# Byshx/Poccala

Hardware: AMD Instinct MI355X
Metric: frames/sec GMM-score+fwd-bwd, 39-d MFCC, 2048-mix (higher is better)
Workload: dtype f32-class (f16x2 split operands, f32 accumulate; f64 dynamic programming)

## Files before the change

### poccala_amd/csrc/batch_plan.h

```cpp
#pragma once
#include <math.h>
#include <stdint.h>

#include <algorithm>
#include <vector>

#include "pcl_own.h"

struct ScoreSeg {
    long long frame0;
    long long out0;
    int len;
    int out_stride;
    int vstart;
    int pad;
};
struct DupRow {
    long long src, dst;
    int T, N;
};
struct ScoreTile {
    int state;
    int seg_lo, seg_hi;
    int vstart;
// ... 119 lines not shown

template <typename Rows>
static int plan_sparse_trans(pcl_ctx *ctx, const char *who, std::vector<UttDesc> &utt, Rows rows, SparseTrans *out) {
    SparseTrans s;
    size_t np = 0;
    for (const UttDesc &d : utt) np += (size_t)d.N + 1;
    s.row_ptr.resize(np);
    s.col_ptr.resize(np);
    std::vector<int> nnz_off(utt.size()), fill;
    for (size_t u = 0; u < utt.size(); ++u) {
        const UttDesc &d = utt[u];
        const int N = d.N;
        const size_t base = s.col_idx.size();
        nnz_off[u] = (int)base;
        int *rp = s.row_ptr.data() + d.ptr_off, *cp = s.col_ptr.data() + d.ptr_off;
        for (int i = 0; i < N; ++i) {
            rp[i] = (int)(s.col_idx.size() - base);
            rows((int)u, i, [&](int j, double v) {
                s.col_idx.push_back(j);
                s.csr_val.push_back(v);
                if (j != i && j != i + 1) s.shape.left_right = false;
            });
            s.shape.max_outdeg = std::max(s.shape.max_outdeg, (int)(s.col_idx.size() - base) - rp[i]);
        }
        if (s.col_idx.size() > 0x7fffffffULL) PCL_FAIL(ctx, PCL_ERR_INVALID, "%s: too many transitions", who);
        const int cnt = rp[N] = (int)(s.col_idx.size() - base);
        std::fill(cp, cp + N + 1, 0);
        for (int k = 0; k < cnt; ++k) ++cp[s.col_idx[base + k] + 1];
        for (int j = 0; j < N; ++j) {
            s.shape.max_indeg = std::max(s.shape.max_indeg, cp[j + 1]);
            cp[j + 1] += cp[j];
        }
        fill.assign(cp, cp + N);
        s.row_idx.resize(base + cnt);
        s.csc_val.resize(base + cnt);
        for (int i = 0; i < N; ++i)
            for (int k = rp[i]; k < rp[i + 1]; ++k) {
                const int q = fill[s.col_idx[base + k]]++;
                s.row_idx[base + q] = i;
                s.csc_val[base + q] = s.csr_val[base + k];
            }
    }
    s.shape.nnz = (long long)s.col_idx.size();
    for (size_t u = 0; u < utt.size(); ++u) utt[u].nnz_off = nnz_off[u];
    *out = std::move(s);
    return PCL_OK;
}

static auto dense_trans_rows(const std::vector<UttDesc> &utt, const double *logA) {
    return [&utt, logA](int u, int i, auto emit) {
        const int N = utt[u].N;
        const double *row = logA + utt[u].mat_off + (size_t)i * N;
        for (int j = 0; j < N; ++j)
            if (!(row[j] == -INFINITY)) emit(j, row[j]);
    };
}
static auto label_trans_rows(const std::vector<UttDesc> &utt, const LabelPlan &lab, const double *unit_logtrans, int S) {
    return [&utt, &lab, unit_logtrans, S](int u, int i, auto emit) {
        if (i == utt[u].N - 1) return;
        const int e = S - 2, p = (i == 0) ? 0 : (i - 1) / e, r = (i == 0) ? 0 : 1 + (i - 1) % e;
        const double *row = unit_logtrans + ((size_t)lab.labels[lab.label_off[u] + p] * S + r) * S;
        for (int c = 0; c < S; ++c)
            if (!(row[c] == -INFINITY)) emit(p * e + c, row[c]);
    };
}

struct ScorePlan {
    std::vector<int32_t> row_state;
    std::vector<ScoreSeg> segs;
    std::vector<DupRow> dups;
    std::vector<int> seg_of_row;
    std::vector<int> work_states;
    std::vector<int> state_seg_lo, state_seg_hi;
    std::vector<int> state_seg_hip;
    int n_segs = 0;
    int max_state = -1;
    int max_N = 0;
};

static int plan_score(pcl_ctx *ctx, const std::vector<UttDesc> &utt, const int32_t *row_state, int J, ScorePlan *out) {
    const int U = (int)utt.size();
    ScorePlan p;
    std::vector<int> start((size_t)J + 1, 0);
    std::vector<long long> frames(J, 0);
    size_t sumN = 0;
    for (int u = 0; u < U; ++u) {
        const UttDesc &d = utt[u];
        for (int n = 0; n < d.N; ++n) {
            const int st = row_state[d.vec_off + n];
            if (st >= J || st < PCL_ROW_EXIT) PCL_FAIL(ctx, PCL_ERR_INVALID, "pcl_batch_set_states: utterance %d row %d has state %d outside [0,%d)", u, n, st, J);
            if (st < 0) continue;
            if (d.frame0 < 0) PCL_FAIL(ctx, PCL_ERR_STATE, "pcl_batch_set_states: batch was created without frame_begin");
            if ((frames[st] += d.T) > 0x7fffffffLL) PCL_FAIL(ctx, PCL_ERR_INVALID, "pcl_batch_set_states: state %d has too many frames", st);
            ++start[st + 1];
            p.max_state = std::max(p.max_state, st);
        }
        sumN += d.N;
        p.max_N = std::max(p.max_N, d.N);
    }
    for (int j = 0; j < J; ++j) start[j + 1] += start[j];
    p.n_segs = start[J];
    p.row_state.assign(row_state, row_state + sumN);
    std::vector<int> nprim(J, 0), first_row(J, -1), touched;
    std::vector<char> is_dup(sumN, 0);
    for (int u = 0; u < U; ++u) {
        const UttDesc &d = utt[u];
        touched.clear();
        for (int n = 0; n < d.N; ++n) {
            const int st = row_state[d.vec_off + n];
            if (st < 0) continue;
            if (first_row[st] < 0) {
                first_row[st] = n;
                touched.push_back(st);
                ++nprim[st];
            } else {
                is_dup[d.vec_off + n] = 1;
                p.dups.push_back(DupRow{d.b_off + first_row[st], d.b_off + n, d.T, d.N});
            }
        }
        for (int st : touched) first_row[st] = -1;
    }
    p.segs.assign(p.n_segs, ScoreSeg());
    p.seg_of_row.assign(sumN, -1);
    std::vector<int> fill(start.begin(), start.end() - 1);
    std::fill(frames.begin(), frames.end(), 0);
    for (int pass = 0; pass < 2; ++pass)
        for (int u = 0; u < U; ++u) {
            const UttDesc &d = utt[u];
            for (int n = 0; n < d.N; ++n) {
                const int st = row_state[d.vec_off + n];
                if (st < 0 || (int)is_dup[d.vec_off + n] != pass) continue;
                p.seg_of_row[d.vec_off + n] = fill[st];
                ScoreSeg &s = p.segs[fill[st]++];
                s.frame0 = d.frame0;
                s.out0 = d.b_off + n;
                s.len = d.T;
                s.out_stride = d.N;
                s.vstart = (int)frames[st];
                s.pad = st;
                frames[st] += d.T;
            }
        }
    for (int j = 0; j < J; ++j)
        if (start[j + 1] > start[j]) {
            p.work_states.push_back(j);
            p.state_seg_lo.push_back(start[j]);
            p.state_seg_hi.push_back(start[j + 1]);
            p.state_seg_hip.push_back(start[j] + nprim[j]);
        }
    *out = std::move(p);
    return PCL_OK;
}

static std::vector<ScoreTile> plan_tiles(const ScorePlan &p, const std::vector<size_t> &which, int tf) {
    constexpr int NXCD = 8;
    std::vector<ScoreTile> queue[NXCD];
    std::vector<long long> load(NXCD, 0);
    for (size_t k : which) {
        const int lo = p.state_seg_lo[k], hi = p.state_seg_hip[k];
        const long long tot = (long long)p.segs[hi - 1].vstart + p.segs[hi - 1].len;
        int g = 0;
        for (int x = 1; x < NXCD; ++x)
            if (load[x] < load[g]) g = x;
        int s0 = lo;
        for (long long v = 0; v < tot; v += tf) {
            while (s0 + 1 < hi && p.segs[s0 + 1].vstart <= v) ++s0;
            queue[g].push_back(ScoreTile{p.work_states[k], lo, hi, (int)v, s0});
        }
        load[g] += (tot + tf - 1) / tf;
    }
    size_t depth = 0;
    for (int x = 0; x < NXCD; ++x) depth = std::max(depth, queue[x].size());
    std::vector<ScoreTile> tiles;
    tiles.reserve(depth * NXCD);
    for (size_t q = 0; q < depth; ++q)
        for (int x = 0; x < NXCD; ++x) tiles.push_back(q < queue[x].size() ? queue[x][q] : ScoreTile{0, 0, 0, 0, 0});
    return tiles;
}
```

### poccala_amd/csrc/pcl_api.hip

```cpp
#include <math.h>
#include <stdio.h>
#include <stdlib.h>
#include <string.h>

#include <algorithm>

#include <map>
#include <memory>
#include <mutex>
#include <unordered_map>

#include "pcl_internal.h"

static std::string g_init_error;

void pcl_set_error(pcl_ctx *ctx, const char *msg) {
    if (ctx) ctx->err = msg;
    else g_init_error = msg;
}

void pcl_timer_begin(pcl_ctx *ctx, const char *which) {
    if (!ctx->timing) return;
    TimedEventPair p;
    if (p.make() != hipSuccess) return;
// ... 24 lines not shown
size_t pool_class(size_t n) {
    if (n <= 256) return 256;
    size_t p2 = 256;
    while (p2 < n) p2 <<= 1;
    if (p2 <= (1u << 20)) return p2;
    const size_t step = p2 >> 4;
    return (n + step - 1) / step * step;
}
size_t pool_limit() {
    static const size_t lim = (size_t)(getenv("PCL_POOL_MAX_MB") ? atol(getenv("PCL_POOL_MAX_MB")) : 65536) << 20;
    return lim;
}
void pool_release_locked(size_t keep) {
    while (g_pool_cached > keep && !g_pool_free.empty()) {
        auto best = g_pool_free.begin();
        for (auto it = g_pool_free.begin(); it != g_pool_free.end(); ++it)
            if (it->first.second > best->first.second) best = it;
        int cur = 0;
        (void)hipGetDevice(&cur);
        if (cur != best->first.first) (void)hipSetDevice(best->first.first);
        (void)hipFree(best->second);
        if (cur != best->first.first) (void)hipSetDevice(cur);
        g_pool_cached -= best->first.second;
        g_pool_live.erase(best->second);
        g_pool_free.erase(best);
    }
}
}

void *pcl_pool_alloc(int device, size_t bytes) {
    const size_t cls = pool_class(bytes);
    std::lock_guard<std::mutex> lock(g_pool_mu);
    auto it = g_pool_free.find(std::make_pair(device, cls));
    if (it != g_pool_free.end()) {
        void *p = it->second;
        g_pool_free.erase(it);
        g_pool_cached -= cls;
        return p;
    }
    void *p = nullptr;
    if (hipMalloc(&p, cls) != hipSuccess) {
        (void)hipGetLastError();
        pool_release_locked(0);
        if (hipMalloc(&p, cls) != hipSuccess) {
            (void)hipGetLastError();
            return nullptr;
        }
    }
    ++g_pool_device_allocs;
    g_pool_live[p] = PoolBlock{cls, device};
    return p;
}

void pcl_pool_free(void *p) {
    if (!p) return;
    const bool wait = pcl_tls_free_synced <= 0;
    if (wait) (void)hipDeviceSynchronize();
    std::lock_guard<std::mutex> lock(g_pool_mu);
    if (wait) ++g_pool_device_waits;
    auto it = g_pool_live.find(p);
    if (it == g_pool_live.end()) {
        (void)hipFree(p);
        return;
    }
    g_pool_free.emplace(std::make_pair(it->second.device, it->second.bytes), p);
    g_pool_cached += it->second.bytes;
    if (g_pool_cached > pool_limit()) pool_release_locked(pool_limit() / 2);
}

extern "C" int pcl_pool_stats(size_t *handed_out_blocks, size_t *handed_out_bytes, size_t *cached_bytes, uint64_t *device_allocs, uint64_t *device_waits) {
    std::lock_guard<std::mutex> lock(g_pool_mu);
    size_t live_bytes = 0;
    for (const auto &kv : g_pool_live) live_bytes += kv.second.bytes;
    if (handed_out_blocks) *handed_out_blocks = g_pool_live.size() - g_pool_free.size();
    if (handed_out_bytes) *handed_out_bytes = live_bytes - g_pool_cached;
    if (cached_bytes) *cached_bytes = g_pool_cached;
    if (device_allocs) *device_allocs = g_pool_device_allocs;
    if (device_waits) *device_waits = g_pool_device_waits;
    return PCL_OK;
}

namespace {
__global__ void desc_copy_kernel(DescCopyArgs a, const char *__restrict__ stage) {
    const int e = blockIdx.y;
    if (e >= a.n) return;
    const unsigned long long n = a.bytes[e];
    if (n == 0) return;
    const char *src = stage + a.off[e];
    char *dst = (char *)a.dst[e];
    const unsigned long long n16 = n / 16;
    for (unsigned long long i = blockIdx.x * (unsigned long long)blockDim.x + threadIdx.x; i < n16; i += (unsigned long long)gridDim.x * blockDim.x)
        ((uint4 *)dst)[i] = ((const uint4 *)src)[i];
    if (blockIdx.x == 0)
        for (unsigned long long i = n16 * 16 + threadIdx.x; i < n; i += blockDim.x) dst[i] = src[i];
}
}

hipError_t pcl_desc_launch(pcl_ctx *ctx, const DescCopyArgs &a, const char *pin) {
    void *dev_stage = nullptr;
    hipError_t e = hipHostGetDevicePointer(&dev_stage, const_cast<char *>(pin), 0);
    if (e != hipSuccess) return e;
    hipLaunchKernelGGL(desc_copy_kernel, dim3(32, a.n), dim3(256), 0, ctx->stream_desc, a, (const char *)dev_stage);
    e = hipGetLastError();
    return e != hipSuccess ? e : hipStreamSynchronize(ctx->stream_desc);
}

static int pcl_batch_reap(pcl_ctx *ctx, bool wait);

extern "C" {

static void free_model(pcl_ctx *ctx) {
    pcl_accumulate_release(ctx);
    pcl_coarse_release(ctx);
    ctx->nbad.clear();
    if (ctx->zero_pending && ctx->ev_zero) (void)hipEventSynchronize(ctx->ev_zero);
    ctx->zero_pending = false;
    static_cast<ModelDev &>(*ctx) = {};
    ctx->st_acc = ctx->st_alpha = ctx->st_mean = ctx->st_cov = nullptr;
    ctx->J = ctx->M = ctx->Mpad = 0;
}

static void release_frames32(pcl_ctx *ctx) {
    if (ctx->frames_front < 0) ctx->frames_up.release();
    ctx->frames32 = nullptr;
    ctx->frames_front = -1;
}

static int ctx_setup(pcl_ctx *ctx) {
    HIPCHK(nullptr, hipSetDevice(ctx->device));
    hipDeviceProp_t prop;
    if (hipGetDeviceProperties(&prop, ctx->device) == hipSuccess) ctx->cus = prop.multiProcessorCount;
    HIPCHK(nullptr, ctx->stream_main.make(StreamKind::Plain));
    ctx->stream = ctx->stream_main;
    HIPCHK(nullptr, ctx->stream_dp.make(StreamKind::HighPriority));
    HIPCHK(nullptr, ctx->stream_aux.make(StreamKind::Plain));
    HIPCHK(nullptr, ctx->stream_desc.make(StreamKind::NonBlocking));
    HIPCHK(nullptr, ctx->stream_d2h.make(StreamKind::NonBlocking));
    const char *var = getenv("PCL_SCORE_VARIANT");
    ctx->score_variant = var ? atoi(var) : 7;
    if (ctx->score_variant != 1 && ctx->score_variant != 3 && ctx->score_variant != 7)
        PCL_FAIL(nullptr, PCL_ERR_INVALID, "pcl_init: PCL_SCORE_VARIANT must be 1, 3 or 7");
    if (const char *cm = getenv("PCL_MFMA_COND_MAX")) ctx->cond_max = (float)atof(cm);
    if (const char *sm = getenv("PCL_SPLIT_MAX")) {
        ctx->split_frac = std::min(1.0f, std::max(0.0f, (float)atof(sm)));
        ctx->split_frac_set = true;
    }
    if (const char *ds = getenv("PCL_DP_STREAM")) ctx->dp_async = atoi(ds) != 0;
    if (const char *co = getenv("PCL_COARSE")) ctx->coarse_on = atoi(co) != 0;
    if (const char *cm2 = getenv("PCL_COMPACT_MAIN")) ctx->compact_main = atoi(cm2) != 0;
    if (const char *cs = getenv("PCL_COARSE_STATS")) ctx->coarse_stats = atoi(cs) != 0;
    if (const char *cp = getenv("PCL_COARSE_PASSES")) ctx->coarse_np = atoi(cp) == 3 ? 3 : 1;
    if (const char *cm_ = getenv("PCL_COARSE_SPLIT_MAX")) ctx->coarse_split_frac = std::min(1.0f, std::max(0.0f, (float)atof(cm_)));
    if (const char *tm = getenv("PCL_TIMERS")) ctx->timing = atoi(tm) != 0;
    return PCL_OK;
}

static void ctx_teardown(pcl_ctx *ctx) {
    pcl_comm_destroy(ctx);
    pcl_batch_reap(ctx, true);
    ctx->zero_pending = false;
    delete ctx;
}

int pcl_init(int device, pcl_ctx **out) {
    if (!out) PCL_FAIL(nullptr, PCL_ERR_INVALID, "pcl_init: out is NULL");
    *out = nullptr;
    setenv("GPU_MAX_HW_QUEUES", "8", 0);
    int n = 0;
    hipError_t e = hipGetDeviceCount(&n);
    if (e != hipSuccess || n == 0)
        PCL_FAIL(nullptr, PCL_ERR_HIP, "pcl_init: no HIP device (%s)", e == hipSuccess ? "count = 0" : hipGetErrorString(e));
    if (device < 0 || device >= n) PCL_FAIL(nullptr, PCL_ERR_INVALID, "pcl_init: device %d out of range [0,%d)", device, n);
    pcl_ctx *ctx = new pcl_ctx();
    ctx->device = device;
    const int rc = ctx_setup(ctx);
    if (rc != PCL_OK) {
        ctx_teardown(ctx);
        return rc;
    }
    *out = ctx;
    return PCL_OK;
}

int pcl_destroy(pcl_ctx *ctx) {
    if (!ctx) return PCL_OK;
    hipSetDevice(ctx->device);
    for (int round = 0; round < 2; ++round) {
        for (hipStream_t s : ctx->streams())
            if (s) hipStreamSynchronize(s);
    }
    ctx_teardown(ctx);
    return PCL_OK;
}

const char *pcl_last_error(pcl_ctx *ctx) { return ctx ? ctx->err.c_str() : g_init_error.c_str(); }

static int sync_main_and_dp(pcl_ctx *ctx) {
    HIPCHK(ctx, hipStreamSynchronize(ctx->stream));
    HIPCHK(ctx, hipStreamSynchronize(ctx->stream_dp));
    return PCL_OK;
}

int pcl_sync(pcl_ctx *ctx) {
    if (!ctx) return PCL_ERR_INVALID;
    TRY(sync_main_and_dp(ctx));
    HIPCHK(ctx, hipStreamSynchronize(ctx->stream_aux));
    if (ctx->stream_d2h) HIPCHK(ctx, hipStreamSynchronize(ctx->stream_d2h));
    pcl_batch_reap(ctx, false);
    return PCL_OK;
}

static int batch_join(pcl_batch *b) {
    if (b->dp_pending) {
        HIPCHK(b->ctx, hipStreamWaitEvent(b->ctx->stream, b->ev_dp, 0));
        b->dp_pending = false;
    }
    if (b->fetch_pending) {
        HIPCHK(b->ctx, hipStreamWaitEvent(b->ctx->stream, b->ev_fetch, 0));
        b->fetch_pending = false;
    }
    return PCL_OK;
}

int pcl_device_info(pcl_ctx *ctx, char *name, int cap, int *cus, size_t *hbm_bytes) {
    if (!ctx) return PCL_ERR_INVALID;
    hipDeviceProp_t prop;
    HIPCHK(ctx, hipGetDeviceProperties(&prop, ctx->device));
    if (name && cap > 0) snprintf(name, cap, "%s (%s)", prop.name, prop.gcnArchName);
    if (cus) *cus = prop.multiProcessorCount;
    if (hbm_bytes) *hbm_bytes = prop.totalGlobalMem;
    return PCL_OK;
}

int pcl_timing_enable(pcl_ctx *ctx, int on) {
    if (!ctx) return PCL_ERR_INVALID;
    TRY(sync_main_and_dp(ctx));
    if (!on) ctx->timers.clear();
    ctx->timing = on != 0;
    return PCL_OK;
}

int pcl_kernel_time(pcl_ctx *ctx, const char *which, float *total_ms, int *launches) {
    if (!ctx || !which) return PCL_ERR_INVALID;
    TRY(sync_main_and_dp(ctx));
    float tot = 0.f;
    int n = 0;
    auto it = ctx->timers.find(which);
    if (it != ctx->timers.end()) {
        for (auto &p : it->second.ev) {
            float ms = 0.f;
            if (hipEventElapsedTime(&ms, p.first, p.second) == hipSuccess) {
                tot += ms;
                ++n;
            }
        }
        it->second.ev.clear();
        tot += (float)it->second.host_ms;
        n += it->second.host_n;
        it->second.host_ms = 0.0;
        it->second.host_n = 0;
    }
    if (total_ms) *total_ms = tot;
    if (launches) *launches = n;
    return PCL_OK;
}

static int device_dim(int D) {
    const int pipe[] = {13, 26, 39, 47};
    for (int o : pipe)
        if (D <= o) return o;
    const int opts[] = {48, 64};
    for (int o : opts)
        if (D <= o) return o;
    return -1;
}

int pcl_device_dim(int D) { return device_dim(D); }

void pcl_frames_adopt(pcl_ctx *ctx, DevBuf<float> &&f32, DevBuf<double> &&f64, int64_t F, int D) {
    release_frames32(ctx);
    ctx->frames64.release();
    ctx->frames_up = std::move(f32);
    ctx->frames32 = ctx->frames_up;
    ctx->frames64 = std::move(f64);
    ctx->F = F;
    ctx->FD = device_dim(D);
    ctx->FDhost = D;
    if (ctx->fmllr_Gk && D != ctx->Dhost) pcl_fmllr_release(ctx);
    if (ctx->mllt_F && D != ctx->Dhost) pcl_mllt_release(ctx);
}

int pcl_model_alloc(pcl_ctx *ctx, int J, int M, int D, int flags, const char *who) {
    if (J <= 0 || M <= 0 || D <= 0) PCL_FAIL(ctx, PCL_ERR_INVALID, "%s: bad shape J=%d M=%d D=%d", who, J, M, D);
    const int Dd = device_dim(D);
    if (Dd < 0) PCL_FAIL(ctx, PCL_ERR_INVALID, "%s: feature dimension %d > 64 is not supported", who, D);
    HIPCHK(ctx, hipSetDevice(ctx->device));
    free_model(ctx);
    const int Mpad = (M + 3) / 4 * 4;
    const int row = (2 * Dd + 1 + 3) / 4 * 4;
    const int Mp32 = (M + 31) / 32 * 32, KS4 = (Dd + 1 + 3) / 4;
    const size_t nm = (size_t)J * Mpad * Dd, nw = (size_t)J * Mpad;
    const size_t npm = (size_t)J * (Mp32 / 32) * KS4 * 64 * 4;
    TRY(ctx->mean64.alloc(ctx, nm));
    TRY(ctx->var64.alloc(ctx, nm));
    TRY(ctx->w64.alloc(ctx, nw));
    TRY(ctx->pm32.alloc(ctx, npm));
// ... 228 lines not shown
    else ctx->graves.push_back(b);
    return PCL_OK;
}

int pcl_batch_upload_sparse(pcl_batch *b, const SparseTrans &t, const double *logpi) {
    pcl_ctx *ctx = b->ctx;
    b->trans = t.shape;
    b->row_ptr.release(); b->col_idx.release(); b->csr_val.release();
    b->col_ptr.release(); b->row_idx.release(); b->csc_val.release();
    b->xi_m.release(); b->xi_s.release(); b->nz_tmp.release();
    const size_t nz = (size_t)t.shape.nnz, np = t.row_ptr.size();
    TRY(b->row_ptr.alloc(ctx, np));
    TRY(b->col_ptr.alloc(ctx, np));
    TRY(b->col_idx.alloc(ctx, nz));
    TRY(b->row_idx.alloc(ctx, nz));
    TRY(b->csr_val.alloc(ctx, nz));
    TRY(b->csc_val.alloc(ctx, nz));
    TRY(b->xi_m.alloc(ctx, nz));
    TRY(b->xi_s.alloc(ctx, nz));
    auto up = b->launched ? pcl_h2d : pcl_h2d_fresh;
    HIPCHK(ctx, up(ctx, b->row_ptr, t.row_ptr.data(), np * sizeof(int)));
    HIPCHK(ctx, up(ctx, b->col_ptr, t.col_ptr.data(), np * sizeof(int)));
    if (nz) {
        HIPCHK(ctx, up(ctx, b->col_idx, t.col_idx.data(), nz * sizeof(int)));
        HIPCHK(ctx, up(ctx, b->row_idx, t.row_idx.data(), nz * sizeof(int)));
        HIPCHK(ctx, up(ctx, b->csr_val, t.csr_val.data(), nz * sizeof(double)));
        HIPCHK(ctx, up(ctx, b->csc_val, t.csc_val.data(), nz * sizeof(double)));
    }
    HIPCHK(ctx, up(ctx, b->logpi, logpi, (size_t)b->shape.sumN * sizeof(double)));
    HIPCHK(ctx, up(ctx, b->d_utt, b->shape.utt.data(), (size_t)b->U * sizeof(UttDesc)));
    b->have_trans = true;
    b->have_fb = b->have_vit = false;
    return PCL_OK;
}

int pcl_batch_set_transitions(pcl_batch *b, const double *logA, const double *logpi) {
    if (!b) return PCL_ERR_INVALID;
    pcl_ctx *ctx = b->ctx;
    TRY(batch_join(b));
    if (!logA || !logpi) PCL_FAIL(ctx, PCL_ERR_INVALID, "pcl_batch_set_transitions: NULL argument");
    HIPCHK(ctx, hipSetDevice(ctx->device));
    SparseTrans t;
    TRY(plan_sparse_trans(ctx, "pcl_batch_set_transitions", b->shape.utt, dense_trans_rows(b->shape.utt, logA), &t));
    return pcl_batch_upload_sparse(b, t, logpi);
}

int pcl_batch_set_states(pcl_batch *b, const int32_t *row_state) {
    if (!b) return PCL_ERR_INVALID;
    TRY(batch_join(b));
    if (!row_state) PCL_FAIL(b->ctx, PCL_ERR_INVALID, "pcl_batch_set_states: NULL argument");
    return pcl_batch_set_states_impl(b, row_state);
}

int pcl_batch_set_states_impl(pcl_batch *b, const int32_t *row_state) {
    pcl_ctx *ctx = b->ctx;
    if (ctx->J == 0) PCL_FAIL(ctx, PCL_ERR_STATE, "pcl_batch_set_states: upload a model first");
    HIPCHK(ctx, hipSetDevice(ctx->device));
    ScorePlan plan;
    TRY(plan_score(ctx, b->shape.utt, row_state, ctx->J, &plan));
    b->plan = std::move(plan);
    b->d_dups.release();
    if (!b->plan.dups.empty()) {
        TRY(b->d_dups.alloc(ctx, b->plan.dups.size()));
        HIPCHK(ctx, pcl_h2d_fresh(ctx, b->d_dups, b->plan.dups.data(), b->plan.dups.size() * sizeof(DupRow)));
    }
    b->d_segs.release();
    b->d_tiles.release();
    b->d_tiles_v.release();
    b->d_tiles_s.release();
    b->d_tiles_c.release();
    b->d_tile_flags_c.release();
    b->n_tiles_s = b->n_tiles_c = 0;
    b->tile_frames = 0;
    TRY(b->d_segs.alloc(ctx, (size_t)b->plan.n_segs));
    if (b->plan.n_segs) HIPCHK(ctx, pcl_h2d_fresh(ctx, b->d_segs, b->plan.segs.data(), (size_t)b->plan.n_segs * sizeof(ScoreSeg)));
    b->d_seg_of_row.release();
    TRY(b->d_seg_of_row.alloc(ctx, (size_t)b->shape.sumN));
    if (b->shape.sumN) HIPCHK(ctx, pcl_h2d_fresh(ctx, b->d_seg_of_row, b->plan.seg_of_row.data(), (size_t)b->shape.sumN * sizeof(int)));
    auto up = b->launched ? pcl_h2d : pcl_h2d_fresh;
    HIPCHK(ctx, up(ctx, b->d_row_state, row_state, (size_t)b->shape.sumN * sizeof(int32_t)));
    HIPCHK(ctx, up(ctx, b->d_utt, b->shape.utt.data(), (size_t)b->U * sizeof(UttDesc)));
    b->have_states = true;
    b->virt_rows_filled = false;
    b->model_J = ctx->J;
    return PCL_OK;
}

static int batch_revalidate(pcl_batch *b, const char *who) {
    pcl_ctx *ctx = b->ctx;
    if (b->shape.max_frame_end > ctx->F)
        PCL_FAIL(ctx, PCL_ERR_STATE, "%s: the batch refers to frame rows up to %lld but the frame matrix now has %lld rows (re-uploaded after the batch was created)",
                 who, b->shape.max_frame_end, (long long)ctx->F);
    if (b->have_states && (b->plan.max_state >= ctx->J || b->model_J != ctx->J))
        PCL_FAIL(ctx, PCL_ERR_STATE, "%s: the batch was laid out for a model of %d states (largest id used %d) but the model now has %d (re-uploaded after pcl_batch_set_states)",
                 who, b->model_J, b->plan.max_state, ctx->J);
    return PCL_OK;
}

static int ensure_tmp(pcl_batch *b) {
    if (!b->tmp) TRY(b->tmp.alloc(b->ctx, (size_t)b->shape.sumNT));
    return PCL_OK;
}

int pcl_batch_set_emissions(pcl_batch *b, const double *B) {
    if (!b) return PCL_ERR_INVALID;
    pcl_ctx *ctx = b->ctx;
    TRY(batch_join(b));
    if (!B) PCL_FAIL(ctx, PCL_ERR_INVALID, "pcl_batch_set_emissions: NULL argument");
    HIPCHK(ctx, hipSetDevice(ctx->device));
    TRY(ensure_tmp(b));
    b->launched = true;
    HIPCHK(ctx, pcl_h2d(ctx, b->d_utt, b->shape.utt.data(), (size_t)b->U * sizeof(UttDesc)));
    HIPCHK(ctx, hipMemcpyAsync(b->tmp, B, (size_t)b->shape.sumNT * sizeof(double), hipMemcpyHostToDevice, ctx->stream));
    TRY(pcl_launch_transpose(ctx, b, b->tmp, b->Bt, 1));
    HIPCHK(ctx, hipStreamSynchronize(ctx->stream));
    b->have_B = true;
    b->virt_rows_filled = false;
    b->have_fb = b->have_vit = false;
    return PCL_OK;
}

int pcl_batch_set_posteriors(pcl_batch *b, const double *lgamma) {
    if (!b) return PCL_ERR_INVALID;
    pcl_ctx *ctx = b->ctx;
    TRY(batch_join(b));
    if (!lgamma) PCL_FAIL(ctx, PCL_ERR_INVALID, "pcl_batch_set_posteriors: NULL argument");
    HIPCHK(ctx, hipSetDevice(ctx->device));
    TRY(ensure_tmp(b));
    if (!b->lgam) TRY(b->lgam.alloc(ctx, (size_t)b->shape.sumNT));
    HIPCHK(ctx, pcl_h2d(ctx, b->d_utt, b->shape.utt.data(), (size_t)b->U * sizeof(UttDesc)));
    HIPCHK(ctx, hipMemcpyAsync(b->tmp, lgamma, (size_t)b->shape.sumNT * sizeof(double), hipMemcpyHostToDevice, ctx->stream));
    TRY(pcl_launch_transpose(ctx, b, b->tmp, b->lgam, 1));
    HIPCHK(ctx, hipStreamSynchronize(ctx->stream));
    b->have_post = true;
    return PCL_OK;
}

static int ensure_frames64(pcl_ctx *ctx) {
    if (ctx->frames64 || !ctx->frames32) return PCL_OK;
    const size_t n = (size_t)ctx->F * ctx->FD;
    TRY(ctx->frames64.alloc(ctx, n));
    return pcl_launch_cast(ctx, nullptr, ctx->frames32, ctx->frames64, n);
}

static int build_tiles(pcl_batch *b, int precision) {
    pcl_ctx *ctx = b->ctx;
    const int route = pcl_route(ctx, precision, ctx->D);
    const bool mfma = route != PCL_ROUTE_DIRECT;
    const int tf = route == PCL_ROUTE_SPLIT16 ? pcl_score_split16_tile_frames()
                 : route == PCL_ROUTE_MFMA32 ? pcl_score_mfma_tile_frames() : pcl_score_tile_frames(ctx->D, precision);
    if (b->d_tiles && b->tile_frames == tf && b->tile_gen == ctx->model_gen) return PCL_OK;
    std::vector<size_t> good, bad;
    for (size_t k = 0; k < b->plan.work_states.size(); ++k) (mfma && pcl_state_uses_valu(ctx, b->plan.work_states[k]) ? bad : good).push_back(k);
    const std::vector<ScoreTile> tiles = plan_tiles(b->plan, good, tf);
    const std::vector<ScoreTile> tiles_v = bad.empty() ? std::vector<ScoreTile>() : plan_tiles(b->plan, bad, pcl_score_tile_frames(ctx->D, PCL_F32));
    std::vector<size_t> split;
    if (mfma)
        for (size_t k : good)
            if (pcl_state_is_split(ctx, b->plan.work_states[k])) split.push_back(k);
    const bool coarse = route == PCL_ROUTE_SPLIT16 && pcl_coarse_enabled(ctx);
    const std::vector<ScoreTile> tiles_s = (split.empty() || coarse) ? std::vector<ScoreTile>() : plan_tiles(b->plan, split, pcl_score_subset_tile_frames(ctx->D));
    const std::vector<ScoreTile> tiles_c = (split.empty() || !coarse) ? std::vector<ScoreTile>() : plan_tiles(b->plan, split, pcl_coarse_tile_frames());
    b->d_tiles.release();
    b->d_tiles_v.release();
    b->d_tiles_s.release();
    b->d_tiles_c.release();
    b->d_tile_flags_c.release();
    pcl_desc_group uploads(ctx);
    b->n_tiles_s = (int)tiles_s.size();
    if (!tiles_s.empty()) {
        TRY(b->d_tiles_s.alloc(ctx, tiles_s.size()));
        HIPCHK(ctx, pcl_h2d_fresh(ctx, b->d_tiles_s, tiles_s.data(), tiles_s.size() * sizeof(ScoreTile)));
    }
    b->n_tiles_c = (int)tiles_c.size();
    if (!tiles_c.empty()) {
        TRY(b->d_tiles_c.alloc(ctx, tiles_c.size()));
        TRY(b->d_tile_flags_c.alloc(ctx, tiles_c.size()));
        HIPCHK(ctx, pcl_h2d_fresh(ctx, b->d_tiles_c, tiles_c.data(), tiles_c.size() * sizeof(ScoreTile)));
    }
    b->d_tile_flags.release();
    TRY(b->d_tile_flags.alloc(ctx, tiles.size()));
    b->n_tiles = (int)tiles.size();
    b->n_tiles_v = (int)tiles_v.size();
    b->tile_frames = tf;
    b->tile_gen = ctx->model_gen;
    TRY(b->d_tiles.alloc(ctx, tiles.size()));
    if (!tiles.empty()) HIPCHK(ctx, pcl_h2d_fresh(ctx, b->d_tiles, tiles.data(), tiles.size() * sizeof(ScoreTile)));
    if (!tiles_v.empty()) {
        TRY(b->d_tiles_v.alloc(ctx, tiles_v.size()));
        HIPCHK(ctx, pcl_h2d_fresh(ctx, b->d_tiles_v, tiles_v.data(), tiles_v.size() * sizeof(ScoreTile)));
    }
    HIPCHK(ctx, uploads.finish());
    return PCL_OK;
}

int pcl_batch_score(pcl_batch *b, int precision) {
    if (!b) return PCL_ERR_INVALID;
    pcl_ctx *ctx = b->ctx;
    TRY(batch_join(b));
    if (precision != PCL_F32 && precision != PCL_F64) PCL_FAIL(ctx, PCL_ERR_INVALID, "pcl_batch_score: precision %d", precision);
    if (ctx->J == 0) PCL_FAIL(ctx, PCL_ERR_STATE, "pcl_batch_score: no model uploaded");
    if (ctx->F == 0) PCL_FAIL(ctx, PCL_ERR_STATE, "pcl_batch_score: no frames uploaded");
    if (!b->have_states) PCL_FAIL(ctx, PCL_ERR_STATE, "pcl_batch_score: pcl_batch_set_states was not called");
    if (ctx->FDhost != ctx->Dhost)
        PCL_FAIL(ctx, PCL_ERR_INVALID, "data dimension %d does not match model dimension %d", ctx->FDhost, ctx->Dhost);
    TRY(batch_revalidate(b, "pcl_batch_score"));
    HIPCHK(ctx, hipSetDevice(ctx->device));
    if (precision == PCL_F64) {
        TRY(ensure_frames64(ctx));
        TRY(pcl_ensure_layouts(ctx, PCL_LAYOUT_P64));
    }
    TRY(build_tiles(b, precision));
    b->launched = true;
    if (!b->virt_rows_filled) {
        TRY(pcl_launch_fill_virtual_rows(ctx, b));
        b->virt_rows_filled = true;
    }
    const int route = pcl_route(ctx, precision, ctx->D);
    if (route != PCL_ROUTE_DIRECT) {
        if (route == PCL_ROUTE_SPLIT16) {
            TRY(pcl_launch_score_split16(ctx, b, b->d_tiles, b->n_tiles));
#ifndef PCL_DIAG_NOFIXUP
            TRY(pcl_launch_score_fixup(ctx, b, b->d_tiles, b->n_tiles, b->d_tile_flags));
#endif
        } else TRY(pcl_launch_score_mfma(ctx, b, b->d_tiles, b->n_tiles));
        if (b->n_tiles_c) {
            TRY(pcl_launch_score_coarse(ctx, b));
            TRY(pcl_launch_score_subset_flagged(ctx, b, b->d_tiles_c, b->n_tiles_c, b->d_tile_flags_c));
        }
        TRY(pcl_launch_score_subset(ctx, b, b->d_tiles_s, b->n_tiles_s));
        TRY(pcl_launch_score(ctx, b, PCL_F32, b->d_tiles_v, b->n_tiles_v));
    } else {
        TRY(pcl_launch_score(ctx, b, precision, b->d_tiles, b->n_tiles));
    }
    TRY(pcl_launch_dup_rows(ctx, b));
    HIPCHK(ctx, pcl_batch_mark(b));
    b->mark_is_score = true;
    b->have_B = true;
    b->have_fb = b->have_vit = false;
    return PCL_OK;
}

int pcl_batch_forward_backward(pcl_batch *b, int fix_pi, double threshold) {
    if (!b) return PCL_ERR_INVALID;
    pcl_ctx *ctx = b->ctx;
    if (!b->have_trans) PCL_FAIL(ctx, PCL_ERR_STATE, "pcl_batch_forward_backward: no transitions set");
    if (!b->have_B) PCL_FAIL(ctx, PCL_ERR_STATE, "pcl_batch_forward_backward: no emissions (score or set_emissions first)");
    HIPCHK(ctx, hipSetDevice(ctx->device));
    const bool after_fetch = b->fetch_pending;
    if (b->fetch_pending) {
        HIPCHK(ctx, hipStreamWaitEvent(ctx->stream, b->ev_fetch, 0));
        b->fetch_pending = false;
    }
    if (!b->alpha) {
        TRY(b->alpha.alloc(ctx, (size_t)b->shape.sumNT));
        TRY(b->beta.alloc(ctx, (size_t)b->shape.sumNT));
        if (!b->lgam) TRY(b->lgam.alloc(ctx, (size_t)b->shape.sumNT));
        TRY(b->pi_out.alloc(ctx, (size_t)b->shape.sumN));
        TRY(b->gamma_out.alloc(ctx, (size_t)b->shape.sumN));
        TRY(b->ksai.alloc(ctx, (size_t)b->shape.sumNN));
        TRY(b->logp.alloc(ctx, (size_t)b->U));
        TRY(b->qtrace.alloc(ctx, (size_t)b->U * PCL_MAX_PASS));
        TRY(b->npass.alloc(ctx, (size_t)b->U));
    }
    if (ctx->dp_async) {
        TRY(pcl_run_on_dp_stream(b, after_fetch, [&] { return pcl_launch_forward_backward(ctx, b, fix_pi ? 1 : 0, threshold); }));
    } else {
        TRY(pcl_launch_forward_backward(ctx, b, fix_pi ? 1 : 0, threshold));
        HIPCHK(ctx, pcl_batch_mark(b));
        b->mark_is_score = false;
    }
    b->have_fb = true;
    b->have_post = true;
    return PCL_OK;
}

int pcl_batch_viterbi(pcl_batch *b, int end_state_back) {
    if (!b) return PCL_ERR_INVALID;
    pcl_ctx *ctx = b->ctx;
    if (!b->have_trans) PCL_FAIL(ctx, PCL_ERR_STATE, "pcl_batch_viterbi: no transitions set");
    if (!b->have_B) PCL_FAIL(ctx, PCL_ERR_STATE, "pcl_batch_viterbi: no emissions (score or set_emissions first)");
    HIPCHK(ctx, hipSetDevice(ctx->device));
    const bool after_fetch = b->fetch_pending;
    if (b->fetch_pending) {
        HIPCHK(ctx, hipStreamWaitEvent(ctx->stream, b->ev_fetch, 0));
        b->fetch_pending = false;
    }
    if (!b->bp) {
        TRY(b->bp.alloc(ctx, (size_t)b->shape.sumNT));
        TRY(b->path.alloc(ctx, (size_t)b->shape.sumT));
        TRY(b->point.alloc(ctx, (size_t)b->U));
    }
    if (ctx->dp_async) {
        TRY(pcl_run_on_dp_stream(b, after_fetch, [&] { return pcl_launch_viterbi(ctx, b, end_state_back ? 1 : 0); }));
    } else {
        TRY(batch_join(b));
        TRY(pcl_launch_viterbi(ctx, b, end_state_back ? 1 : 0));
        HIPCHK(ctx, pcl_batch_mark(b));
        b->mark_is_score = false;
    }
    b->have_vit = true;
    return PCL_OK;
}

int pcl_batch_regroup(pcl_batch *b, const int32_t *row_unit, int gmm_num, int32_t *frame_unit, int32_t *frame_k) {
    if (!b) return PCL_ERR_INVALID;
    pcl_ctx *ctx = b->ctx;
    TRY(batch_join(b));
    if (!row_unit || !frame_unit || !frame_k || gmm_num < 1) PCL_FAIL(ctx, PCL_ERR_INVALID, "pcl_batch_regroup: bad arguments");
    if (!b->have_vit) PCL_FAIL(ctx, PCL_ERR_STATE, "pcl_batch_regroup: run pcl_batch_viterbi first");
    HIPCHK(ctx, hipSetDevice(ctx->device));
    DevBuf<int32_t> d_ru, d_fu, d_fk;
    TRY(d_ru.alloc(ctx, (size_t)b->shape.sumN));
    TRY(d_fu.alloc(ctx, (size_t)b->shape.sumT));
    TRY(d_fk.alloc(ctx, (size_t)b->shape.sumT));
// ... 516 lines not shown
```

### poccala_amd/csrc/pcl_internal.h

```cpp
#pragma once
#include <hip/hip_runtime.h>
#include <stdint.h>
#include <stdlib.h>
#include <string.h>

#include <algorithm>
#include <array>

#include <map>
#include <string>
#include <vector>

#include "../../include/poccala_hip.h"
#include "pcl_own.h"
#include "pcl_desc.h"
#include "batch_plan.h"
#include "frontend_host.h"

struct ActiveFrame {
    long long frame;
    double coef;
    double lg;
};

struct KernelTimer {
    std::vector<TimedEventPair> ev;
    double host_ms = 0.0;
    int host_n = 0;
};

struct PcmStage {
    Stream stream;
    PinBuf<int16_t> pin[2];
    LazyEvent ev[2];
};
struct MfccTables {
    DevBuf<double> d;
    int nfft = 0, nfilt = 0, rank = 0;
    std::vector<double> host;
};

struct AccScratch {
    DevBuf<int> cnt; DevBuf<long long> off; DevBuf<ActiveFrame> list;
    DevBuf<int> work_states, seg_lo, seg_hi, split_flag;
    DevBuf<unsigned char> images[2];
    DevBuf<int> tile_off[2], state_flag[2];
    DevBuf<unsigned int> tile_mask[2];
    LazyEvent ev_prod[2], ev_cons[2], ev_start;
};

struct ModelDev {
    DevBuf<float> params32;
    DevBuf<double> params64;
    DevBuf<float> pm32;
    DevBuf<float> centers32;
    DevBuf<unsigned short> pm16f;
    DevBuf<double> kzero;
    DevBuf<float> fscale;
    DevBuf<float> d_cond;
    DevBuf<unsigned char> d_bad;
    DevBuf<int> d_bad_idx;
    DevBuf<int> d_nbad;
    DevBuf<int> d_non;
    DevBuf<int> d_good_idx;
    DevBuf<int> d_npt;
    DevBuf<float> mean32;
    DevBuf<double> mean64;
    DevBuf<double> var64, w64;
    DevBuf<double> stats;
    DevBuf<double> fmllr_Gk;
    DevBuf<double> fmllr_beta;
    DevBuf<double> fmllr_W;
    DevBuf<double> mllr_W;
    DevBuf<double> ebw_num;
    DevBuf<double> mllt_F;
    DevBuf<double> mllt_beta;
    DevBuf<int> mllt_keep;
    std::vector<int32_t> mllt_keep_host;
};
struct CoarseDev {
    DevBuf<unsigned short> pmc;
    DevBuf<float> fscale_c;
    DevBuf<double> kzero_c;
    DevBuf<float> rows_c;
    DevBuf<float> kgap_c;
    DevBuf<double> k2c;
    DevBuf<int> d_nct;
    DevBuf<unsigned long long> d_coarse_counter;
};
struct UnitsDev {
    DevBuf<double> d_unit_trans;
    DevBuf<double> hmm_ksai;
};
struct LexiconDev {
    DevBuf<int> lex_units, lex_nunits, lex_child_ptr, lex_child_idx, lex_word, lex_roots;
    DevBuf<int4> lex_info;
    DevBuf<double> d_unit_logtrans;
    DevBuf<double> lm_uni, lm_bow, lm_val;
    DevBuf<long long> lm_row_ptr;
    DevBuf<int> lm_col, lm_node_word_ptr, lm_node_word_ids;
    DevBuf<int> lex_tie_gen;
    DevBuf<int4> lex_tie_lr;
};

struct TyingDev {
    DevBuf<int4> ty_nodes;
    DevBuf<unsigned int> ty_qbits;
    DevBuf<int> ty_root;
};

struct CtxStreams {
    Stream stream_main;
    Stream stream_dp;
    Stream stream_aux;
    Stream stream_desc;
    Stream stream_d2h;
    Stream stream_comm;
};

struct pcl_ctx : CtxStreams, ModelDev, CoarseDev, UnitsDev, LexiconDev, TyingDev {
    int device = 0;
    AccScratch acc;
    hipStream_t stream = nullptr;
    std::string err;
    int cus = 0;
    int J = 0, M = 0, Mpad = 0, D = 0, Dhost = 0, row = 0;
    int model_flags = 0;
    int mllr_R = 0;
    int fmllr_S = 0;
    int Mpad32 = 0;
    int layouts_valid = 0;
    bool dp_async = true;
    int score_wgs_per_cu = 0;
    int score_variant = 0;
    std::vector<float> cond;
    float cond_max = 96.f;
    bool compact_main = true;
    std::vector<int> nbad;
    float split_frac = 0.5f;
    bool split_frac_set = false;
    int split_max = 0;
    int model_gen = 0;
    int coarse_np = 1;
    int coarse_gen = -1;
    float coarse_split_frac = 0.99f;
    bool coarse_stats = false;
    bool coarse_on = true;
    int acc_split_max = 0;
    int64_t F = 0;
    int FD = 0, FDhost = 0;
    float *frames32 = nullptr;
    DevBuf<float> frames_up;
    DevBuf<double> frames64;
    int live_batches = 0, live_segs = 0;
    DevBuf<double> lda_stats;
    int lda_R = 0, lda_left = 0, lda_right = 0, lda_D = 0;
    DevBuf<long long> cmvn_n;
    DevBuf<double> cmvn_sq;
    int cmvn_S = 0, cmvn_D = 0;
    DevBuf<double> tree_stats;
    int tree_R = 0, tree_D = 0;
    DevBuf<float> frames_slot[2];
    int frames_front = -1, staged_slot = -1, staged_D = 0;
    int64_t staged_F = 0;
    LazyEvent ev_stage, ev_slot_free;
    bool have_slot_free = false;
    size_t stats_len = 0;
    double *st_acc = nullptr, *st_alpha = nullptr, *st_mean = nullptr, *st_cov = nullptr;
    DevBuf<double> d_softplus;
    bool stats_fresh = false;
    LazyEvent ev_zero, ev_zero_src;
    bool zero_pending = false;
    double acc_prune_log2 = -1e300;
    int n_units = 0, S = 0;
    std::vector<double> unit_trans, unit_logtrans;
    double *hmm_gamma = nullptr;
    int lex_nodes = 0, lex_nroots = 0;
    std::vector<int> lex_word_host;
    std::vector<int> lex_units_host, lex_nunits_host;
    int lex_tie_Jt = 0, lex_tie_P = 0;
    int lm_W = 0;
    int ty_N = 0, ty_Q = 0, ty_W = 0, ty_R0 = 0, ty_Jt = 0, ty_P = 0, ty_units = 0;
    void *comm = nullptr;
    int rank = 0, nranks = 1;
    int transport = 0;
    pcl_allgather_fn host_allgather = nullptr;
    void *host_user = nullptr;
    DevBuf<float> payload32;
    std::vector<LazyEvent> pipe_ev;
    LazyEvent pipe_done;
    bool pipe_active = false;
    int pipe_early = 0;
    int pipe_K = 0, pipe_next = 0, pipe_payload = 0, pipe_mode = 1;
    double pipe_c_cov = 0.0;
    std::map<std::string, KernelTimer> timers;
    bool timing = false;
    std::vector<struct pcl_batch *> graves;
    DescStager<> desc;
    PcmStage pcm;
    MfccTables mfcc_tab;
    std::array<hipStream_t, 7> streams() const { return {stream_main, stream_dp, stream_aux, stream_d2h, stream_desc, stream_comm, pcm.stream}; }
};

struct BatchDecodeDev {
    DevBuf<double> dec_f64;
    DevBuf<int> dec_slot, dec_work, dec_int;
    DevBuf<double> dec_score;
    int dec_cap = 0, dec_cand = 0, dec_nodes = 0;
    DevBuf<int> dec_word;
    bool dec_has_words = false;
};

struct pcl_batch : BatchDecodeDev {
    pcl_ctx *ctx = nullptr;
    int U = 0;
    BatchShape shape;
    TransShape trans;
    ScorePlan plan;
    LabelPlan lab;
    int model_J = 0;
    bool have_trans = false, have_states = false, have_B = false, have_fb = false, have_vit = false, have_post = false;
    bool launched = false;
    bool virt_rows_filled = false;
    DevBuf<UttDesc> d_utt;
    DevBuf<double> Bt, alpha, beta, lgam;
    DevBuf<double> logpi, pi_out, gamma_out, ksai;
    DevBuf<double> logp, qtrace, point;
    DevBuf<int32_t> npass, path;
    DevBuf<int> row_ptr, col_idx;
    DevBuf<double> csr_val;
    DevBuf<int> col_ptr, row_idx;
    DevBuf<double> csc_val;
    DevBuf<double> xi_m, xi_s;
    DevBuf<unsigned long long> Bp;
    DevBuf<int> alpha_e, beta_e, fb_kmax;
    DevBuf<double> fb_dump;
    DevBuf<double> fb_part_m;
    DevBuf<int> fb_part_e;
    bool fb_linear = false;
    DevBuf<unsigned short> bp;
    DevBuf<int32_t> d_row_state;
    DevBuf<ScoreSeg> d_segs;
    DevBuf<DupRow> d_dups;
    DevBuf<ScoreTile> d_tiles;
    std::vector<int> acc_ws, acc_lo, acc_hi, acc_split;
    LazyEvent ev_main, ev_dp;
    bool mark_is_score = false;
    LazyEvent ev_mark;
    bool dp_pending = false;
    LazyEvent ev_fetch, ev_fetch_src;
    bool fetch_pending = false;
    DevBuf<int> d_tile_flags;
    DevBuf<ScoreTile> d_tiles_v;
    DevBuf<ScoreTile> d_tiles_s;
    DevBuf<ScoreTile> d_tiles_c;
    DevBuf<int> d_tile_flags_c;
    int n_tiles_c = 0;
    int n_tiles = 0, n_tiles_v = 0, n_tiles_s = 0, tile_frames = 0, tile_gen = -1;
    DevBuf<double> tmp;
    DevBuf<double> nz_tmp;
    DevBuf<int> d_seg_of_row;
    bool counted = false;
    bool have_dec = false;
    bool from_labels = false;
    std::vector<double> logpi_u;
    DevBuf<int> occ_ptr, occ_utt, occ_row0;
    DevBuf<int32_t> d_labels;
    DevBuf<int> d_label_off;
    bool tied = false;
    int tied_J = 0;
    DevBuf<int32_t> pos_state;
};

struct FbPassRule {
    struct Verdict { bool final_pass, q6; };
    const bool fix_pi;
    const double threshold;
    double q = -INFINITY;
    int npass = 0;
    __device__ __forceinline__ FbPassRule(int fix_pi_, double threshold_) : fix_pi(fix_pi_ != 0), threshold(threshold_) {}
    __device__ __forceinline__ Verdict judge(double qnew) const {
        const bool natural = !(qnew - q > threshold) || (npass + 1 >= PCL_MAX_PASS);
        const bool q6 = fix_pi && !natural && threshold >= 0.0 && npass + 1 < PCL_MAX_PASS;
        return {natural || q6, q6};
    }
    __device__ __forceinline__ void record(Verdict v, double qnew, double *__restrict__ trace, bool writer) {
        if (writer) trace[npass] = qnew;
// ... 242 lines not shown
```

Before: 22.47 million.

## Group states with identical segment layouts into cohorts placed together per XCD

The tile planner now sorts work states by their segment layout (frame0, len, vstart) and groups identical-layout states into cohorts of up to PCL_COHORT_MAX. Each cohort, or a chunk that fits a per-XCD slot budget, goes to one XCD with tiles interleaved frame-major, so neighbouring workgroups read the same frame tiles. The aim is better L2 reuse of frame data on each XCD. In exchange, load balancing becomes coarser and tile order changes, and a new env knob bounds the cohort size.

```diff
diff --git a/poccala_amd/csrc/batch_plan.h b/poccala_amd/csrc/batch_plan.h
--- a/poccala_amd/csrc/batch_plan.h
+++ b/poccala_amd/csrc/batch_plan.h
@@ -295,22 +295,71 @@
     return PCL_OK;
 }
 
-static std::vector<ScoreTile> plan_tiles(const ScorePlan &p, const std::vector<size_t> &which, int tf) {
+#ifndef PCL_COHORT_MAX
+#define PCL_COHORT_MAX 4
+#endif
+static std::vector<std::vector<size_t>> plan_cohorts(const ScorePlan &p, const std::vector<size_t> &which, int cohort_max = PCL_COHORT_MAX) {
+    const auto cmp = [&p](size_t a, size_t b) {
+        const int la = p.state_seg_lo[a], lb = p.state_seg_lo[b], na = p.state_seg_hip[a] - la, nb = p.state_seg_hip[b] - lb;
+        if (na != nb) return na < nb ? -1 : 1;
+        for (int s = 0; s < na; ++s) {
+            const ScoreSeg &x = p.segs[la + s], &y = p.segs[lb + s];
+            if (x.frame0 != y.frame0) return x.frame0 < y.frame0 ? -1 : 1;
+            if (x.len != y.len) return x.len < y.len ? -1 : 1;
+            if (x.vstart != y.vstart) return x.vstart < y.vstart ? -1 : 1;
+        }
+        return 0;
+    };
+    std::vector<size_t> order(which);
+    std::sort(order.begin(), order.end(), [&](size_t a, size_t b) {
+        const int c = cmp(a, b);
+        return c ? c < 0 : a < b;
+    });
+    std::vector<std::vector<size_t>> cohorts;
+    const size_t cap = (size_t)std::max(cohort_max, 1);
+    for (size_t i = 0; i < order.size(); ++i) {
+        if (i == 0 || cmp(order[i - 1], order[i]) != 0 || cohorts.back().size() >= cap) cohorts.emplace_back();
+        cohorts.back().push_back(order[i]);
+    }
+    std::sort(cohorts.begin(), cohorts.end(), [](const std::vector<size_t> &a, const std::vector<size_t> &b) { return a[0] < b[0]; });
+    return cohorts;
+}
+
+#ifndef PCL_XCD_SLOTS
+#define PCL_XCD_SLOTS 96
+#endif
+static std::vector<ScoreTile> plan_tiles(const ScorePlan &p, const std::vector<size_t> &which, int tf, int cohort_max = PCL_COHORT_MAX) {
     constexpr int NXCD = 8;
     std::vector<ScoreTile> queue[NXCD];
     std::vector<long long> load(NXCD, 0);
-    for (size_t k : which) {
-        const int lo = p.state_seg_lo[k], hi = p.state_seg_hip[k];
-        const long long tot = (long long)p.segs[hi - 1].vstart + p.segs[hi - 1].len;
+    const auto n_tiles = [&](size_t k) {
+        const int hi = p.state_seg_hip[k];
+        return ((long long)p.segs[hi - 1].vstart + p.segs[hi - 1].len + tf - 1) / tf;
+    };
+    const auto least_loaded = [&]() {
         int g = 0;
         for (int x = 1; x < NXCD; ++x)
             if (load[x] < load[g]) g = x;
-        int s0 = lo;
-        for (long long v = 0; v < tot; v += tf) {
-            while (s0 + 1 < hi && p.segs[s0 + 1].vstart <= v) ++s0;
-            queue[g].push_back(ScoreTile{p.work_states[k], lo, hi, (int)v, s0});
-        }
-        load[g] += (tot + tf - 1) / tf;
+        return g;
+    };
+    const auto place = [&](const std::vector<size_t> &c, size_t m0, size_t m1, int g) {
+        const long long nt = n_tiles(c[m0]);
+        std::vector<int> s0(m1 - m0);
+        for (size_t m = m0; m < m1; ++m) s0[m - m0] = p.state_seg_lo[c[m]];
+        for (long long i = 0; i < nt; ++i)
+            for (size_t m = m0; m < m1; ++m) {
+                const size_t k = c[m];
+                const int lo = p.state_seg_lo[k], hi = p.state_seg_hip[k];
+                const long long v = i * tf;
+                int &s = s0[m - m0];
+                while (s + 1 < hi && p.segs[s + 1].vstart <= v) ++s;
+                queue[g].push_back(ScoreTile{p.work_states[k], lo, hi, (int)v, s});
+            }
+        load[g] += nt * (long long)(m1 - m0);
+    };
+    for (const std::vector<size_t> &c : plan_cohorts(p, which, cohort_max)) {
+        const size_t fit = (size_t)std::max(1LL, PCL_XCD_SLOTS / n_tiles(c[0]));
+        for (size_t m = 0; m < c.size(); m += fit) place(c, m, std::min(c.size(), m + fit), least_loaded());
     }
     size_t depth = 0;
     for (int x = 0; x < NXCD; ++x) depth = std::max(depth, queue[x].size());
diff --git a/poccala_amd/csrc/pcl_api.hip b/poccala_amd/csrc/pcl_api.hip
--- a/poccala_amd/csrc/pcl_api.hip
+++ b/poccala_amd/csrc/pcl_api.hip
@@ -200,6 +200,7 @@
     if (const char *cp = getenv("PCL_COARSE_PASSES")) ctx->coarse_np = atoi(cp) == 3 ? 3 : 1;
     if (const char *cm_ = getenv("PCL_COARSE_SPLIT_MAX")) ctx->coarse_split_frac = std::min(1.0f, std::max(0.0f, (float)atof(cm_)));
     if (const char *tm = getenv("PCL_TIMERS")) ctx->timing = atoi(tm) != 0;
+    if (const char *ch = getenv("PCL_COHORT_MAX")) ctx->cohort_max = std::min(PCL_COHORT_MAX, std::max(1, atoi(ch)));
     return PCL_OK;
 }
 
@@ -734,15 +735,16 @@
     if (b->d_tiles && b->tile_frames == tf && b->tile_gen == ctx->model_gen) return PCL_OK;
     std::vector<size_t> good, bad;
     for (size_t k = 0; k < b->plan.work_states.size(); ++k) (mfma && pcl_state_uses_valu(ctx, b->plan.work_states[k]) ? bad : good).push_back(k);
-    const std::vector<ScoreTile> tiles = plan_tiles(b->plan, good, tf);
-    const std::vector<ScoreTile> tiles_v = bad.empty() ? std::vector<ScoreTile>() : plan_tiles(b->plan, bad, pcl_score_tile_frames(ctx->D, PCL_F32));
+    const int cmax = ctx->cohort_max;
+    const std::vector<ScoreTile> tiles = plan_tiles(b->plan, good, tf, cmax);
+    const std::vector<ScoreTile> tiles_v = bad.empty() ? std::vector<ScoreTile>() : plan_tiles(b->plan, bad, pcl_score_tile_frames(ctx->D, PCL_F32), cmax);
     std::vector<size_t> split;
     if (mfma)
         for (size_t k : good)
             if (pcl_state_is_split(ctx, b->plan.work_states[k])) split.push_back(k);
     const bool coarse = route == PCL_ROUTE_SPLIT16 && pcl_coarse_enabled(ctx);
-    const std::vector<ScoreTile> tiles_s = (split.empty() || coarse) ? std::vector<ScoreTile>() : plan_tiles(b->plan, split, pcl_score_subset_tile_frames(ctx->D));
-    const std::vector<ScoreTile> tiles_c = (split.empty() || !coarse) ? std::vector<ScoreTile>() : plan_tiles(b->plan, split, pcl_coarse_tile_frames());
+    const std::vector<ScoreTile> tiles_s = (split.empty() || coarse) ? std::vector<ScoreTile>() : plan_tiles(b->plan, split, pcl_score_subset_tile_frames(ctx->D), cmax);
+    const std::vector<ScoreTile> tiles_c = (split.empty() || !coarse) ? std::vector<ScoreTile>() : plan_tiles(b->plan, split, pcl_coarse_tile_frames(), cmax);
     b->d_tiles.release();
     b->d_tiles_v.release();
     b->d_tiles_s.release();
diff --git a/poccala_amd/csrc/pcl_internal.h b/poccala_amd/csrc/pcl_internal.h
--- a/poccala_amd/csrc/pcl_internal.h
+++ b/poccala_amd/csrc/pcl_internal.h
@@ -133,6 +133,7 @@
     bool dp_async = true;
     int score_wgs_per_cu = 0;
     int score_variant = 0;
+    int cohort_max = PCL_COHORT_MAX;
     std::vector<float> cond;
     float cond_max = 96.f;
     bool compact_main = true;
```

Result: no change. 22.37 million (-0.4%).
